# TianyiFranklinWang/MIRROR

Hardware: AMD Instinct MI355X
Metric: SSL samples/sec (slide+RNA pairs) (higher is better)
Workload: dtype bf16; 1 GPU; BASELINE c2: B=16/GPU x [4096 patch tokens x 1024-d] + [2048 genes], D=512, RNA depth 6 / 8 heads, train mode, local-batch InfoNCE; precision_policy=bf16, per_gpu_batch=16, global_batch=16, parallelism=dp1, grad_bucket_dtype=f32, step_launch=hip_graph

## Files before the change

include/mirror_hip.h:

```cpp
#ifndef MIRROR_HIP_H
#define MIRROR_HIP_H
#include <stdint.h>

#ifdef __cplusplus
extern "C" {
#endif

#define MH_OK 0
#define MH_EINVAL (-1)
#define MH_EUNSUP (-2)
#define MH_EHIP (-3)

#define MH_F32 0
#define MH_BF16 1

#define MH_ACT_NONE 0
#define MH_ACT_RELU 1
#define MH_ACT_GELU 2

typedef void* mh_stream;

const char* mh_last_error(void);
int mh_version(void);
int mh_exp_build(void);
// ... 95 lines not shown
                        int dt_x, int dt_dy, int dt_dx, int accumulate_dx, float* workspace, int64_t ws_floats,
                        const void* gadd, int pad, int l, void* relu_out, int relu_first, int relu_rows, float* relu_db,
                        const float* row_mask, const float* lm_scale, mh_stream s);

int mh_quant_fp8(const void* x, int64_t n, void* q, float* scale, unsigned* amax_scratch, int dt, mh_stream s);
int mh_quant_fp8_delayed(const void* x, int64_t n, void* q, float* scale, unsigned* ring, const float* tick, float margin,
                         int dt, mh_stream s);
int mh_gemm_fp8(const void* A, int64_t lda, int64_t a_bs, const void* B, int64_t ldb, void* C, int64_t ldc, int64_t c_bs, int batch,
                const float* scale_a, const float* scale_b, const float* bias, int act, int M, int N, int K, int dt_c, mh_stream s);

int mh_softmax_fwd(const void* x, void* y, int64_t rows, int cols, int64_t ldx, int64_t ldy,
                   int dt_x, int dt_y, mh_stream s);
int mh_softmax_bwd(const void* y, const void* dy, void* dx, int64_t rows, int cols, int64_t ldy, int64_t lddy,
                   int64_t lddx, int dt_y, int dt_dy, int dt_dx, mh_stream s);

int mh_softmax_masked_fwd(const void* x, void* y, const float* rowmask, const float* colmask, int64_t batches, int h, int R,
                          int cols, int dt_x, int dt_y, mh_stream s);
int mh_softmax_masked_bwd(const void* y, const void* dy, void* dx, const float* rowmask, const float* colmask, int64_t batches,
                          int h, int R, int cols, int dt_y, int dt_d, mh_stream s);
int mh_row_scale(const void* x, const float* scale, void* y, int64_t rows, int D, int dt, mh_stream s);
int mh_keymask_plan(const unsigned char* mask, float* mrow, float* mlm, float* lscale, int64_t B, int64_t n_src, int lead, int wrap,
                    int pad, int l, mh_stream s);

int mh_landmark_fwd(const void* qkv, void* lm, int B, int n_p, int D, int l, int dt, mh_stream s);
int mh_landmark_bwd(const void* dlm, void* dqkv, int B, int n_p, int D, int l, int dt, mh_stream s);
int mh_resconv_fwd(const void* v, int64_t ldv, int64_t v_bs, const float* w, void* out, int64_t ldo, int64_t o_bs,
                   int B, int n_p, int heads, int dh, int taps, int transpose, int accumulate,
                   int dt_v, int dt_o, mh_stream s);
int mh_resconv_wgrad(const void* v, int64_t ldv, int64_t v_bs, const void* dout, int64_t ldo, int64_t o_bs,
                     float* dw, int B, int n_p, int heads, int dh, int taps, int dt_v, int dt_o, mh_stream s);
int64_t mh_resconv_bwd_workspace_bytes(int B, int n_p, int heads, int dh, int taps);
int mh_resconv_bwd(const void* dout, int64_t ldo, int64_t o_bs, const void* v, int64_t ldv, int64_t v_bs, const float* w, void* dv,
                   int64_t lddv, int64_t dv_bs, float* dw, float* workspace, int64_t ws_floats, int B, int n_p, int heads, int dh,
                   int taps, int dt_v, int dt_o, mh_stream s);
int mh_pinv_absmax(const float* x, uint64_t* stats64, int BH, int m, mh_stream s);
int mh_pinv_z0(const float* x, const uint64_t* stats64, float* z0, int BH, int m, mh_stream s);
int mh_pinv_z0_bwd(const float* x, const float* z0, const float* dz0, const uint64_t* stats64, float* dx,
                   float* scratch1, int scratch_zeroed, int BH, int m, mh_stream s);
int mh_pinv_s2_bwd(const float* p, const float* dz0, const uint64_t* stats64, float* dx, float* scratch1, int scratch_zeroed, int BH,
                   int m, const float* mlm, int heads, mh_stream s);
int mh_pinv_chain_prep(const float* x, const uint64_t* stats64, float* z0, void* xp, void* z0p, int BH, int m, mh_stream s);
int mh_pinv_chain_pack(const float* dz, void* up, int BH, int m, mh_stream s);
int mh_pinv_chain_fwd(const void* XP, void* saved, void* zfT, int BH, int m, int iters, const float* z0f, const uint64_t* stats64,
                      int z0_rowmajor, mh_stream s);
int mh_nys_sim2(const void* lm, float* a2, void* xp, float* z0f, uint64_t* stats64, int B, int m, int D, int heads, float scale,
                int64_t lm_ld, const float* mlm, mh_stream s);
int mh_nys_dz_dav(const float* dw2, const float* av, const void* zfT, void* up, void* dav, float* delta3, int BH, int m, int dh,
                  mh_stream s);
int mh_pinv_chain_bwd(const void* XP, const void* saved, const void* dzf, void* work, float* dX, float* dz0, int BH, int m,
                      int iters, mh_stream s);
int64_t mh_pinv_chain_workspace_bytes(int BH, int m, int iters, int which);
int mh_nys_attn1_fwd(const void* qkv, const void* lm, const void* w2, void* out, float* lse1, const float* mrow, const float* mlm,
                     int B, int h, int n_p, int m, int dh, float scale, int accumulate, int64_t lm_ld, void* o1, mh_stream s);
int mh_nys_attn1_fwd_q8(const void* qkv, const void* lm, const void* w2, void* out, float* lse1, int B, int h, int n_p, int m, int dh,
                        float scale, int accumulate, void* q8, unsigned* ring, const float* tick, float margin, float* q8_scale, void* o1,
                        mh_stream s);
int64_t mh_nys_attn3_ws_floats(int B, int h, int n_p);
int64_t mh_nys_attn3_workspace_bytes(int B, int h, int n_p);
int mh_nys_attn3_fwd(const void* qkv, const void* lm, float* av, float* lse3, float* workspace, int64_t ws_floats,
                     const float* mrow, const float* mlm, int B, int h, int n_p, int m, int dh, float scale, int64_t lm_ld,
                     const float* rc_w, void* rc_out, mh_stream s);
int mh_nys_attn1_bwd(const void* qkv, const void* lm, const void* w2, const void* dout, const float* lse1, const void* o1, float* delta1,
                     void* dqkv, float* dw2, float* dlm, const float* mrow, const float* mlm, int B, int h, int n_p, int m, int dh,
                     float scale, int64_t lm_ld, mh_stream s);
int mh_nys_attn3_bwd(const void* qkv, const void* lm, const float* av, const void* dav, const float* lse3, float* delta3,
                     void* dqkv, float* dlm, const float* mrow, const float* mlm, int B, int h, int n_p, int m, int dh,
                     float scale, int64_t lm_ld, mh_stream s);
int mh_nys_cls_attn(const void* qkv, const void* lm, const void* z, const float* lse3, float* row, const float* mrow, const float* mlm,
                    int B, int h, int n_p, int m, int dh, int cls_row, float scale, int64_t lm_ld, int z_colmajor, int dt,
                    mh_stream s);
int mh_lm_merge(const float* a, const float* b, void* out, int64_t rows, int cols, int64_t out_ld, int zero_cols, mh_stream s);
int mh_eye_minus(const float* P, float* T, float d, int BH, int m, mh_stream s);

int mh_seq_finish(void* seq, const float* cls, int B, int N, int add, int D, int dt, mh_stream s);
int mh_seq_finish_bwd(void* dseq, float* dcls, int B, int N, int add, int D, int dt, mh_stream s);
int mh_ppeg_merge(const float* w7, const float* w5, const float* w3, const float* b7, const float* b5,
                  const float* b3, float* merged, float* bsum, int D, mh_stream s);
int mh_ppeg_fwd(const void* x, void* y, const float* merged, const float* bsum, int B, int S, int D,
                int flip, int dt_x, int dt_y, mh_stream s);
int mh_ppeg_wgrad(const void* x, const void* dout, float* dmerged, float* dbsum, int B, int S, int D,
                  int dt_x, int dt_o, mh_stream s);
int mh_ppeg_bwd(const float* x, const float* dy, const float* merged, float* dx, float* dmerged, float* dbsum, int B, int S,
                int D, void* drop_out, float* drop_db, float p, uint64_t seed, uint64_t offset, const uint64_t* dev_base,
                mh_stream s);
int mh_ppeg_grad_scatter(const float* dmerged, const float* dbsum, float* dw7, float* dw5, float* dw3, float* db7,
                         float* db5, float* db3, int D, mh_stream s);

int mh_rank_mask(const float* noise, float* mask, int B, int N, int len_keep, mh_stream s);
int mh_mask_apply_fwd(const void* x, void* y, const float* mask, const float* token, const float* pos, int B, int T, int D,
                      int first, int token_scalar, int dt_x, int dt_y, mh_stream s);
int mh_mask_apply_bwd_dbias_ok(const void* dy, const void* dx, const float* dpos, int D, int dt_dy, int dt_dx);
int mh_mask_apply_bwd(const void* dy, void* dx, const float* mask, float* dtoken, float* dpos, int B, int T, int D,
                      int first, int token_scalar, int dt_dy, int dt_dx, float* dbias, mh_stream s);

typedef struct {
    int32_t B, D, Hh, H;
    float eps, p_drop;
    uint64_t seed, offset;
    const uint64_t* dev_base;
    const void *w_qkv, *w_proj, *w_fc1, *w_fc2;
    const void *wt_qkv, *wt_proj, *wt_fc1, *wt_fc2;
    const float *b_qkv, *b_proj, *b_fc1, *b_fc2;
    const float *g1, *be1, *g2, *be2;
    const float* x;
    float* y;
    float* stats;
// ... 217 lines not shown
```

mirror_amd/_lib.py:

```python
from __future__ import annotations

import ctypes as C
import os

_HERE = os.path.dirname(os.path.abspath(__file__))
LIB_PATH = os.environ.get("MIRROR_HIP_LIB") or os.path.join(_HERE, "lib", "libmirror_hip.so")

MH_F32, MH_BF16 = 0, 1
ACT_NONE, ACT_RELU, ACT_GELU = 0, 1, 2


class GemmEpi(C.Structure):
    _fields_ = [
        ("kind", C.c_int32), ("resid", C.c_void_p),
        ("p", C.c_float), ("seed", C.c_uint64), ("offset", C.c_uint64), ("dev_base", C.c_void_p),
        ("mask", C.c_void_p), ("token", C.c_void_p), ("pos", C.c_void_p),
        ("rows_per_batch", C.c_int32), ("first", C.c_int32),
        ("tgt", C.c_void_p), ("tgt_bs", C.c_int64), ("sq", C.c_void_p),
    ]


class SkinnyWgradItem(C.Structure):
    _fields_ = [("dy", C.c_void_p), ("lddy", C.c_int64), ("x", C.c_void_p), ("ldx", C.c_int64), ("dw", C.c_void_p), ("lddw", C.c_int64),
                ("db", C.c_void_p), ("M", C.c_int32), ("N", C.c_int32), ("K", C.c_int32), ("dt_dy", C.c_int32), ("dt_x", C.c_int32)]
# ... 53 lines not shown
        ("g_total", C.c_void_p), ("g_terms", C.c_void_p),
        ("d_wsi_emb", C.c_void_p), ("d_rna_emb", C.c_void_p), ("d_logit_scale", C.c_void_p), ("d_align_ext", C.c_void_p),
        ("d_rna_pred", C.c_void_p), ("d_rna_tgt", C.c_void_p), ("d_w_mu", C.c_void_p), ("d_w_logstd", C.c_void_p), ("d_r_mu", C.c_void_p),
        ("d_r_logstd", C.c_void_p), ("d_w_score", C.c_void_p), ("d_r_score", C.c_void_p),
    ]


class RnaBlockDesc(C.Structure):
    _fields_ = (
        [("B", C.c_int32), ("D", C.c_int32), ("Hh", C.c_int32), ("H", C.c_int32), ("eps", C.c_float), ("p_drop", C.c_float),
         ("seed", C.c_uint64), ("offset", C.c_uint64), ("dev_base", C.c_void_p)]
        + [(n, C.c_void_p) for n in (
            "w_qkv", "w_proj", "w_fc1", "w_fc2", "wt_qkv", "wt_proj", "wt_fc1", "wt_fc2",
            "b_qkv", "b_proj", "b_fc1", "b_fc2", "g1", "be1", "g2", "be2",
            "x", "y", "stats", "qkv", "attn", "o", "x1", "u", "f", "dy", "dx",
            "dw_qkv", "dw_proj", "dw_fc1", "dw_fc2", "db_qkv", "db_proj", "db_fc1", "db_fc2", "dg1", "dbe1", "dg2", "dbe2",
            "scratch")])


_SIGS = {
    "mh_gemm": [C.POINTER(GemmDesc)],
    "mh_skinny_fwd": [P, L, P, L, P, P, L, P, L, I, I, I, I, I, I],
    "mh_skinny_wgrad": [P, L, P, L, P, L, P, I, I, I, I, I, I],
    "mh_skinny_wgrad_many": [C.POINTER(SkinnyWgradItem), I],
    "mh_transpose_bf16": [P, P, I, I],
    "mh_transpose_bf16_many": [P, P, P, I, I, I, I],
    "mh_layernorm_fwd": [P, P, P, P, P, P, I, I, I, L, L, F, I, I],
    "mh_layernorm_fwd_dual": [P, P, P, P, P, P, P, I, I, I, L, L, F],
    "mh_layernorm_fwd_q8": [P, P, P, P, P, P, I, I, I, L, L, F, P, P, P, F, P],
    "mh_layernorm_bwd": [P, P, P, P, P, P, P, P, I, I, I, L, L, I, I, I, I, P, L],
    "mh_layernorm_bwd_fan": [P, P, P, P, P, P, P, P, I, I, I, L, L, I, I, P, L, P, F, P],
    "mh_layernorm_bwd_drop": [P, P, P, P, P, P, P, P, I, I, I, L, L, I, I, P, L, P, F, P, P, F, U64, U64, P, P, I],
    "mh_layernorm_bwd_lm": [P, P, P, P, P, P, P, P, I, I, I, L, L, I, I, I, I, P, L, P, I, I, P, I, I, P, P, P],
    "mh_layernorm_fwd_lm": [P, P, P, P, P, P, P, P, I, I, I, L, I, I, F, P, P],
    "mh_softmax_fwd": [P, P, L, I, L, L, I, I],
    "mh_softmax_bwd": [P, P, P, L, I, L, L, L, I, I, I],
    "mh_landmark_fwd": [P, P, I, I, I, I, I],
    "mh_landmark_bwd": [P, P, I, I, I, I, I],
    "mh_resconv_fwd": [P, L, L, P, P, L, L, I, I, I, I, I, I, I, I, I],
    "mh_resconv_wgrad": [P, L, L, P, L, L, P, I, I, I, I, I, I, I],
    "mh_resconv_bwd": [P, L, L, P, L, L, P, P, L, L, P, P, L, I, I, I, I, I, I, I],
    "mh_pinv_absmax": [P, P, I, I],
    "mh_pinv_z0": [P, P, P, I, I],
    "mh_pinv_z0_bwd": [P, P, P, P, P, P, I, I, I],
    "mh_pinv_s2_bwd": [P, P, P, P, P, I, I, I, P, I],
    "mh_eye_minus": [P, P, F, I, I],
    "mh_pinv_chain_prep": [P, P, P, P, P, I, I],
    "mh_pinv_chain_pack": [P, P, I, I],
    "mh_pinv_chain_fwd": [P, P, P, I, I, I, P, P, I],
    "mh_nys_sim2": [P, P, P, P, P, I, I, I, I, F, L, P],
    "mh_nys_dz_dav": [P, P, P, P, P, P, I, I, I],
    "mh_pinv_chain_bwd": [P, P, P, P, P, P, I, I, I],
    "mh_nys_attn1_fwd": [P, P, P, P, P, P, P, I, I, I, I, I, F, I, L, P],
    "mh_nys_attn1_fwd_q8": [P, P, P, P, P, I, I, I, I, I, F, I, P, P, P, F, P, P],
    "mh_nys_attn3_fwd": [P, P, P, P, P, L, P, P, I, I, I, I, I, F, L, P, P],
    "mh_nys_attn1_bwd": [P, P, P, P, P, P, P, P, P, P, P, P, I, I, I, I, I, F, L],
    "mh_nys_attn3_bwd": [P, P, P, P, P, P, P, P, P, P, I, I, I, I, I, F, L],
    "mh_nys_cls_attn": [P, P, P, P, P, P, P, I, I, I, I, I, I, F, L, I, I],
    "mh_seq_finish": [P, P, I, I, I, I, I],
    "mh_seq_finish_bwd": [P, P, I, I, I, I, I],
    "mh_ppeg_merge": [P, P, P, P, P, P, P, P, I],
    "mh_ppeg_fwd": [P, P, P, P, I, I, I, I, I, I],
    "mh_ppeg_wgrad": [P, P, P, P, I, I, I, I, I],
    "mh_ppeg_bwd": [P, P, P, P, P, P, I, I, I, P, P, F, U64, U64, P],
    "mh_ppeg_grad_scatter": [P, P, P, P, P, P, P, P, I],
    "mh_rank_mask": [P, P, I, I, I],
    "mh_mask_apply_fwd": [P, P, P, P, P, I, I, I, I, I, I, I],
    "mh_mask_apply_bwd": [P, P, P, P, P, I, I, I, I, I, I, I, P],
    "mh_headattn_fwd": [P, P, P, I, I, I, I],
    "mh_headattn_bwd": [P, P, P, P, I, I, I, I],
    "mh_add": [P, P, P, L, I, I, I],
    "mh_lm_merge": [P, P, P, L, I, L, I],
    "mh_cast": [P, P, L, I, I],
    "mh_gelu_fwd": [P, P, L, I, I],
    "mh_gelu_bwd": [P, P, P, L, I, I, I],
    "mh_relu_bwd": [P, P, P, L, I, L, L, L, I, I, I],
    "mh_dropout": [P, P, L, F, U64, U64, P, I, I],
    "mh_noise_draws": [P, L, L, U64, U64, P],
    "mh_dropout_add": [P, P, P, L, F, U64, U64, P, I],
    "mh_dropout_lite": [P, P, P, L, F, U64, U64, P, I, I],
    "mh_timestamp": [P],
    "mh_dropout_lite_colsum": [P, P, L, I, F, U64, U64, P, P],
    "mh_colsum": [P, P, L, I, L, I],
    "mh_l2norm_fwd": [P, P, P, I, I, L, F, I, I],
    "mh_l2norm_bwd": [P, P, P, P, I, I, L, F, I, I, I, I],
    "mh_exp_fwd": [P, P, L],
    "mh_exp_bwd": [P, P, P, L, I],
    "mh_reparam_fwd": [P, P, P, P, L],
    "mh_reparam_bwd": [P, P, P, P, P, P, P, L],
    "mh_ce_rows_fwd": [P, L, P, F, I, I, I, F, P, P, P],
    "mh_ce_rows_bwd": [P, L, P, F, P, P, I, F, P, P, I, I, I],
    "mh_mse_masked_fwd": [P, P, P, P, L, I, L, L, I, I],
    "mh_mse_masked_fwd_ordered": [P, P, P, P, L, I, L, L, I, I, P],
    "mh_mse_masked_bwd": [P, P, P, P, P, F, P, P, L, I, L, L, I, I, I, P, I],
    "mh_fanout_bwd": [P, P, F, P, P, I, I, I, I],
    "mh_gather_rows": [P, P, P, L, L, L, I],
    "mh_sample_rows": [P, P, P, P, I, I, L, U64, U64, P, F],
    "mh_sample_weighted": [P, L, P, L, U64, U64, P],
    "mh_quant_fp8": [P, L, P, P, P, I],
    "mh_quant_fp8_delayed": [P, L, P, P, P, P, F, I],
    "mh_gemm_fp8": [P, L, L, P, L, P, L, L, I, P, P, P, I, I, I, I, I],
    "mh_weighted_sum": [P, P, P, P, P, P, F, F, F, F, F, F, I, P],
    "mh_weighted_sum_bwd": [P, F, F, F, F, F, F, I, P],
    "mh_softmax_masked_fwd": [P, P, P, P, L, I, I, I, I, I],
    "mh_softmax_masked_bwd": [P, P, P, P, P, L, I, I, I, I, I],
    "mh_row_scale": [P, P, P, L, I, I],
# ... 145 lines not shown
```

mirror_amd/csrc/nystrom_fused.hip:

```cpp
#include <cstdlib>
#include <cstring>
#include "gemm_kernel.h"

namespace {

constexpr int NM = 256;
constexpr int ND = 64;
constexpr int NP = 72;
constexpr int NT = 256;
constexpr int TR = 128;

typedef __attribute__((address_space(3))) s16x4 lds_s16x4;
typedef short s16x8 __attribute__((ext_vector_type(8)));

__device__ __forceinline__ bf16x8 frag_kc(const bf16_t* img, int row0, int k0, int lane) {
    return *reinterpret_cast<const bf16x8*>(img + (row0 + (lane & 31)) * NP + k0 + 8 * (lane >> 5));
}
template <int PITCH = NP>
__device__ __forceinline__ bf16x8 frag_tr(const bf16_t* img, int col0, int kb, int lane) {
    const int g16 = lane >> 4, i = lane & 15, q = i >> 2, p = i & 3;
    const bf16_t* a0 = img + (kb + 4 * (g16 >> 1) + q) * PITCH + col0 + 16 * (g16 & 1) + 4 * p;
    s16x4 lo = __builtin_amdgcn_ds_read_tr16_b64_v4i16((lds_s16x4*)a0);
    s16x4 hi = __builtin_amdgcn_ds_read_tr16_b64_v4i16((lds_s16x4*)(a0 + 8 * PITCH));
    s16x8 v = __builtin_shufflevector(lo, hi, 0, 1, 2, 3, 4, 5, 6, 7);
// ... 78 lines not shown
__device__ __forceinline__ void tile_store(const u32x4 (&regs)[ROWS * 8 / NT], bf16_t* img, int tid) {
#pragma unroll
    for (int i = 0; i < ROWS * 8 / NT; i++) {
        const int cid = tid + i * NT, r = cid >> 3, c = cid & 7;
        *reinterpret_cast<u32x4*>(img + r * NP + c * 8) = regs[i];
    }
}
__device__ __forceinline__ void store_row8(bf16_t* p, const f32x16& a, int hl) {
    unsigned w[4][2];
#pragma unroll
    for (int g = 0; g < 4; g++) {
        w[g][0] = pack_bf2(a[4 * g + 0], a[4 * g + 1]);
        w[g][1] = pack_bf2(a[4 * g + 2], a[4 * g + 3]);
    }
#pragma unroll
    for (int pr = 0; pr < 2; pr++) {
        const u32x2 s0 = __builtin_amdgcn_permlane32_swap(w[2 * pr][0], w[2 * pr + 1][0], false, false);
        const u32x2 s1 = __builtin_amdgcn_permlane32_swap(w[2 * pr][1], w[2 * pr + 1][1], false, false);
        const u32x4 v = {s0[0], s1[0], s0[1], s1[1]};
        *reinterpret_cast<u32x4*>(p + 8 * (2 * pr + hl)) = v;
    }
}

constexpr float NEG_FILL = -1.0e6f;
__device__ __forceinline__ void mask_fill16(f32x16& l2, const f32x16& vr, float vl) {
#pragma unroll
    for (int e = 0; e < 16; e++) l2[e] = (vr[e] * vl != 0.f) ? l2[e] : NEG_FILL;
}
__device__ __forceinline__ void mask_zero16(f32x16& d, const f32x16& vr, float vl) {
#pragma unroll
    for (int e = 0; e < 16; e++) d[e] = (vr[e] * vl != 0.f) ? d[e] : 0.f;
}

struct Q8Out {
    unsigned char* q;
    unsigned* ring;
    const float* tick;
    float margin;
    float* scale;
};

struct Geo {
    int h, n_p, D;
    float scale, scale2;
    const float* mrow;
    const float* mlm;
    int accumulate;
    long lm_ld;
    const float* rc_w;
    bf16_t* rc_out;
};
constexpr int RC_TAPS = 33, RC_HALO = 16;

template <bool MASKED, bool Q8 = false>
__global__ __launch_bounds__(NT) void nys_a1_fwd_kernel(const bf16_t* __restrict__ qkv, const bf16_t* __restrict__ lm,
                                                        const bf16_t* __restrict__ w2, bf16_t* __restrict__ out,
                                                        float* __restrict__ lse1, Geo g, Q8Out q8 = Q8Out{}, bf16_t* __restrict__ o1 = nullptr) {
    __shared__ __attribute__((aligned(16))) bf16_t s_kl_[NM * NP];
    __shared__ __attribute__((aligned(16))) bf16_t s_w2_[NM * NP];
    __shared__ __attribute__((aligned(16))) float s_mlm_[NM];
    const int tid = threadIdx.x, lane = tid & 63, wave = tid >> 6, c = lane & 31, hl = lane >> 5;
    const int bh = blockIdx.y, b = bh / g.h, hd = bh % g.h, D = g.D;
    const long LD = g.lm_ld;
    float q8mul = 1.f, q8max = 0.f;
    int q8cur = 0;
    if constexpr (Q8) {
        const int t = (int)q8.tick[0];
        q8cur = t % 3;
        const float amax = __uint_as_float(q8.ring[(t + 2) % 3]) * q8.margin;
        q8mul = amax > 0.f ? 448.f / amax : 1.f;
        if (blockIdx.x == 0 && blockIdx.y == 0 && tid == 0) {
            q8.scale[0] = amax > 0.f ? amax / 448.f : 1.f;
            q8.ring[(t + 1) % 3] = 0u;
        }
    }
    stage_rows<NM>(s_kl_, lm + (long)b * NM * LD + D + hd * ND, LD, tid);
    stage_rows<NM>(s_w2_, w2 + (long)bh * NM * ND, ND, tid);
    constexpr bool masked = MASKED;
    s_mlm_[tid] = masked ? g.mlm[(long)b * NM + tid] : 1.f;
    const int nblk = g.n_p / 32, stride = 4 * gridDim.x;
    int rb = 4 * blockIdx.x + wave;
    const bf16_t* qb = qkv + (long)b * g.n_p * 3 * D + hd * ND;
    bf16x8 qn[4];
    if (rb < nblk) {
#pragma unroll
        for (int ks = 0; ks < 4; ks++) qn[ks] = frag_g(qb + (long)(32 * rb + c) * 3 * D, 16 * ks, lane);
    }
    __syncthreads();
#pragma unroll 1
    for (; rb < nblk; rb += stride) {
        const long row = 32L * rb + c;
        int opq = 0;
        asm volatile("" : "+v"(opq));
        const bf16_t* s_kl = s_kl_ + opq;
        const bf16_t* s_w2 = s_w2_ + opq;
        const float* s_mlm = s_mlm_ + opq;
        const float mr = masked ? g.mrow[(long)b * g.n_p + row] : 1.f;
        bf16x8 qf[4];
#pragma unroll
        for (int ks = 0; ks < 4; ks++) qf[ks] = qn[ks];
        if (rb + stride < nblk) {
#pragma unroll
            for (int ks = 0; ks < 4; ks++) qn[ks] = frag_g(qb + (long)(32 * (rb + stride) + c) * 3 * D, 16 * ks, lane);
        }
        bf16_t* orow = out + ((long)b * g.n_p + row) * D + hd * ND;
        u32x2 old[2][4];
        if (g.accumulate) {
#pragma unroll
            for (int nb = 0; nb < 2; nb++)
#pragma unroll
                for (int gq = 0; gq < 4; gq++) old[nb][gq] = *reinterpret_cast<const u32x2*>(orow + 32 * nb + 8 * gq + 4 * hl);
        }
        float mrun = NEG_BIG, lrun = 0.f;
        f32x16 o[2] = {zero16(), zero16()};
        f32x16 snext = zero16();
#pragma unroll
        for (int ks = 0; ks < 4; ks++) snext = MFMA(frag_kc(s_kl, 0, 16 * ks, lane), qf[ks], snext);
#pragma unroll
        for (int blk = 0; blk < 8; blk++) {
            f32x16 sb = snext;
            if (blk + 1 < 8) {
                snext = zero16();
#pragma unroll
                for (int ks = 0; ks < 4; ks++) snext = MFMA(frag_kc(s_kl, 32 * (blk + 1), 16 * ks, lane), qf[ks], snext);
            }
            float sc2 = g.scale2;
            if (masked) {
                sb = sb * g.scale2;
                mask_fill16(sb, rowvals16(s_mlm + 32 * blk, hl), mr);
                sc2 = 1.f;
            }
            float mx = vmax16(sb);
            mx = fmaxf(mx, __shfl_xor(mx, 32, 64));
            const float mnew = fmaxf(mrun, mx * sc2);
            if (__builtin_amdgcn_ballot_w64(mnew != mrun)) {
                const float alpha = __builtin_amdgcn_exp2f(mrun - mnew);
                lrun *= alpha;
                o[0] *= alpha;
                o[1] *= alpha;
                mrun = mnew;
            }
// ... 495 lines not shown
            *reinterpret_cast<u32x2*>(prow + 24) = u32x2{pw1[2], pw1[3]};
            *reinterpret_cast<u32x2*>(drow) = u32x2{dw0[0], dw0[1]};
            *reinterpret_cast<u32x2*>(drow + 8) = u32x2{dw0[2], dw0[3]};
            *reinterpret_cast<u32x2*>(drow + 16) = u32x2{dw1[0], dw1[1]};
            *reinterpret_cast<u32x2*>(drow + 24) = u32x2{dw1[2], dw1[3]};
        }
        __syncthreads();
        if (more) {
            *reinterpret_cast<u32x4*>(s_k + kr * NP + kc * 8) = rk;
            if (tid < HT) s_mr[tid] = masked ? g.mrow[(long)b * g.n_p + (long)(ht + 1) * HT + tid] : 1.f;
        }
        f32x16 a2 = zero16();
#pragma unroll
        for (int t = 0; t < NM / 16; t++) a2 = MFMA(frag_tr(a_img, 32 * dhalf, 16 * t, lane), frag_tr(b_img, 32 * kb2, 16 * t, lane), a2);
        store_row8(dqkv + ((long)b * g.n_p + (long)ht * HT + 32 * kb2 + c) * 3 * D + (isk ? D : 2 * D) + hd * ND + 32 * dhalf, a2, hl);
        __syncthreads();
    }
    float* dqb = dlm + (long)b * NM * 2 * D + hd * ND;
#pragma unroll
    for (int nb = 0; nb < 2; nb++) atomic_tile(dqb + (long)(32 * wave) * 2 * D + 32 * nb, 2 * D, accq[nb], hl, c);
}

int pick_walkers(int BH, int n_p) {
    int w = 1;
    while (BH * w < 512 && 4 * w * 2 <= n_p / 32) w *= 2;
    return w;
}

#define NYS_LAUNCH(kern, grid, block, shm, stream, ...)                                              \
    do {                                                                                             \
        if (g.mrow) hipLaunchKernelGGL((kern<true>), grid, block, shm, stream, __VA_ARGS__);        \
        else hipLaunchKernelGGL((kern<false>), grid, block, shm, stream, __VA_ARGS__);              \
    } while (0)

int check_geo(const char* fn, int B, int h, int n_p, int m, int dh) {
    MH_REQUIRE(m == NM && dh == ND, "%s: built for m = %d landmarks and dh = %d (got m=%d dh=%d); other shapes use mh_gemm + mh_softmax",
               fn, NM, ND, m, dh);
    MH_REQUIRE(B >= 0 && h >= 1 && n_p >= NM && n_p % NM == 0, "%s: n_p=%d must be a positive multiple of %d", fn, n_p, NM);
    return MH_OK;
}

}

extern "C" int mh_nys_attn1_fwd(const void* qkv, const void* lm, const void* w2, void* out, float* lse1, const float* mrow,
                                const float* mlm, int B, int h, int n_p, int m, int dh, float scale, int accumulate, int64_t lm_ld, void* o1,
                                mh_stream s) {
    if (int e = check_geo("mh_nys_attn1_fwd", B, h, n_p, m, dh)) return e;
    MH_REQUIRE(lm_ld == 0 || (lm_ld >= 2L * h * ND && lm_ld % 8 == 0), "mh_nys_attn1_fwd: lm_ld must be 0 or a multiple of 8 >= 2 D");
    if (B == 0) return MH_OK;
    MH_REQUIRE((mrow == nullptr) == (mlm == nullptr), "mh_nys_attn1_fwd: mrow and mlm go together");
    const Geo g{h, n_p, h * ND, scale, scale * LOG2E, mrow, mlm, accumulate, lm_ld > 0 ? lm_ld : 2L * h * ND, nullptr, nullptr};
    MH_REQUIRE((((uintptr_t)o1) & 15) == 0, "mh_nys_attn1_fwd: o1 must be 16-byte aligned");
    NYS_LAUNCH(nys_a1_fwd_kernel, dim3(pick_walkers(B * h, n_p), B * h), dim3(NT), 0, (hipStream_t)s, (const bf16_t*)qkv, (const bf16_t*)lm,
                       (const bf16_t*)w2, (bf16_t*)out, lse1, g, Q8Out{}, (bf16_t*)o1);
    MH_LAUNCH_CHECK("mh_nys_attn1_fwd");
    return MH_OK;
}

extern "C" int mh_nys_attn1_fwd_q8(const void* qkv, const void* lm, const void* w2, void* out, float* lse1, int B, int h, int n_p, int m,
                                   int dh, float scale, int accumulate, void* q8, unsigned* ring, const float* tick, float margin,
                                   float* q8_scale, void* o1, mh_stream s) {
    if (int e = check_geo("mh_nys_attn1_fwd_q8", B, h, n_p, m, dh)) return e;
    if (B == 0) return MH_OK;
    MH_REQUIRE(q8 && ring && tick && q8_scale && margin >= 1.f && ((uintptr_t)q8 & 3) == 0, "mh_nys_attn1_fwd_q8: q8, ring, tick, scale and margin >= 1");
    const Geo g{h, n_p, h * ND, scale, scale * LOG2E, nullptr, nullptr, accumulate, 2L * h * ND, nullptr, nullptr};
    const Q8Out o{(unsigned char*)q8, ring, tick, margin, q8_scale};
    hipLaunchKernelGGL((nys_a1_fwd_kernel<false, true>), dim3(pick_walkers(B * h, n_p), B * h), dim3(NT), 0, (hipStream_t)s, (const bf16_t*)qkv,
                       (const bf16_t*)lm, (const bf16_t*)w2, (bf16_t*)out, lse1, g, o, (bf16_t*)o1);
    MH_LAUNCH_CHECK("mh_nys_attn1_fwd_q8");
    return MH_OK;
}

int pick_splits(int BH, int ntiles);

extern "C" int64_t mh_nys_attn3_ws_floats(int B, int h, int n_p) {
    if (B <= 0 || h <= 0 || n_p < TR) return 0;
    const int splits = pick_splits(B * h, n_p / TR);
    return splits > 1 ? (int64_t)B * h * splits * A3_PART : 0;
}

extern "C" int64_t mh_nys_attn3_workspace_bytes(int B, int h, int n_p) { return 4 * mh_nys_attn3_ws_floats(B, h, n_p); }

extern "C" int mh_nys_attn3_fwd(const void* qkv, const void* lm, float* av, float* lse3, float* workspace, int64_t ws_floats,
                                const float* mrow, const float* mlm, int B, int h, int n_p, int m, int dh, float scale, int64_t lm_ld,
                                const float* rc_w, void* rc_out, mh_stream s) {
    if (int e = check_geo("mh_nys_attn3_fwd", B, h, n_p, m, dh)) return e;
    MH_REQUIRE(lm_ld == 0 || (lm_ld >= 2L * h * ND && lm_ld % 8 == 0), "mh_nys_attn3_fwd: lm_ld must be 0 or a multiple of 8 >= 2 D");
    MH_REQUIRE((rc_w == nullptr) == (rc_out == nullptr) && (((uintptr_t)rc_out) & 15) == 0, "mh_nys_attn3_fwd: rc_w and rc_out (16-byte aligned) go together");
    if (B == 0) return MH_OK;
    const Geo g{h, n_p, h * ND, scale, scale * LOG2E, mrow, mlm, 0, lm_ld > 0 ? lm_ld : 2L * h * ND, rc_w, (bf16_t*)rc_out};
    const int ntiles = n_p / TR;
    int splits = pick_splits(B * h, ntiles);
    if (!workspace || ws_floats < (int64_t)B * h * splits * A3_PART) splits = 1;
    const int tpw = (ntiles + splits - 1) / splits;
    splits = (ntiles + tpw - 1) / tpw;
    if (rc_w) {
        if (g.mrow) hipLaunchKernelGGL((nys_a3_fwd_kernel<true, true>), dim3(splits, B * h), dim3(NT), 0, (hipStream_t)s, (const bf16_t*)qkv,
                                       (const bf16_t*)lm, av, lse3, workspace, g, tpw);
        else hipLaunchKernelGGL((nys_a3_fwd_kernel<false, true>), dim3(splits, B * h), dim3(NT), 0, (hipStream_t)s, (const bf16_t*)qkv,
                                (const bf16_t*)lm, av, lse3, workspace, g, tpw);
    } else {
        NYS_LAUNCH(nys_a3_fwd_kernel, dim3(splits, B * h), dim3(NT), 0, (hipStream_t)s, (const bf16_t*)qkv, (const bf16_t*)lm, av,
                           lse3, workspace, g, tpw);
    }
    MH_LAUNCH_CHECK("mh_nys_attn3_fwd");
    if (splits > 1) {
        hipLaunchKernelGGL(nys_a3_combine_kernel, dim3(ND / 16, B * h), dim3(NM), 0, (hipStream_t)s, (const float*)workspace, av, lse3,
                           splits);
        MH_LAUNCH_CHECK("mh_nys_attn3_fwd(combine)");
    }
    return MH_OK;
}

int pick_splits(int BH, int ntiles) {
    int splits = 1;
    while (BH * splits < 256 && splits * 2 <= ntiles) splits *= 2;
    return splits;
}

extern "C" int mh_nys_attn1_bwd(const void* qkv, const void* lm, const void* w2, const void* dout, const float* lse1, const void* o1,
                                float* delta1, void* dqkv, float* dw2, float* dlm, const float* mrow, const float* mlm, int B, int h,
// ... 32 lines not shown
```

mirror_amd/functional.py:

```python
from __future__ import annotations

from dataclasses import dataclass
from typing import List, Optional, Tuple

import os

import torch
from torch.autograd import Function

from . import kernels as K
from ._lib import ACT_NONE, ACT_RELU, MH_BF16, MH_F32

f32, bf16 = torch.float32, torch.bfloat16


@dataclass(frozen=True)
class Precision:
    name: str
    mma: int
    act: torch.dtype
    pinv_mma: int
    fp8_fwd: bool = False


# ... 1670 lines not shown
                z0, xt = K.pinv_chain_prep(a2, st, K.pinv_chain_z0_slot(chain_saved))
            zfT = torch.empty((Bn, h, m_l, m_l), device=qkv.device, dtype=bf16)
            zf = zfT.transpose(-1, -2)
            side = _side_stream(qkv.device)
            side.wait_stream(torch.cuda.current_stream())
            with torch.cuda.stream(side):
                if one:
                    K.nys_sim2(lm, h, scale, st, out=(a2, xt), mlm=mlm_s2)
                    K.pinv_chain_fwd(xt, chain_saved, zfT, iters, z0f=a2, stats=st, z0_rowmajor=True)
                else:
                    K.pinv_chain_fwd(xt, chain_saved, zfT, iters)
            saved = [(xt, chain_saved, z0 if z0 is not None else st)]
            ctx.z0_stored = z0 is not None
            K.shared_chip = True
        tile = (not chain) and pm == MH_BF16 and K.gemm_tile_ok(m_l, m_l, m_l)
        if tile and _TILE_SIDE:
            side = _side_stream(qkv.device)
            side.wait_stream(torch.cuda.current_stream())
            with torch.cuda.stream(side):
                zf, saved, st, ctx.a2b = pinv_forward_tile(a2, iters, want_a2b=True)
        if link is not None:
            link.core = True
            link.run("v_cols")
        fused = K.nys_fused_ok(qkv, h, m_l) and lm.dtype == bf16
        lse1 = lse3 = a1 = a3 = None
        out = torch.empty((Bn, n_p, D), device=qkv.device, dtype=A)
        rc_in_a3 = fused and _RC_FUSED and A == bf16 and res_w.numel() == h * 33
        if fused:
            av, lse3 = K.nys_attn3_fwd(qkv, lm, h, scale, kmask,
                                       rc=(res_w.detach().reshape(-1).contiguous(), out) if rc_in_a3 else None)
        else:
            sm1 = (kmask is None and A == bf16 and mma == MH_BF16 and q.dtype == bf16
                   and K.gemm_softmax_ok(n_p, lm.shape[1], dh, q.dtype, kl.dtype))
            if sm1:
                a1 = K.gemm(q, kl.transpose(-1, -2), alpha=scale, mma=mma, out_dtype=bf16, softmax=True)
            else:
                a1 = K.gemm(q, kl.transpose(-1, -2), alpha=scale, mma=mma, out_dtype=f32)
            a3 = K.gemm(ql, k.transpose(-1, -2), alpha=scale, mma=mma, out_dtype=f32)
            if kmask is None:
                if not sm1:
                    a1 = K.softmax_fwd(a1, a1 if A == f32 else None, out_dtype=A)
                a3 = K.softmax_fwd(a3, a3 if A == f32 else None, out_dtype=A)
            else:
                a1 = K.softmax_masked_fwd(a1, mrow, mlm, a1 if A == f32 else None, out_dtype=A)
                a3 = K.softmax_masked_fwd(a3, mlm, mrow, a3 if A == f32 else None, out_dtype=A)
        if tile and not _TILE_SIDE:
            zf, saved, st, ctx.a2b = pinv_forward_tile(a2, iters, want_a2b=True)
        elif not chain and not tile:
            zf, saved, st = pinv_forward(a2, iters, pm, sd)
        if not fused:
            av = K.gemm(a3, v, mma=mma, out_dtype=f32)
        pio = pm if (pm == MH_BF16 or A == f32) else mma
        w2 = None
        if side is not None and fused:
            w2 = torch.empty((Bn, h, m_l, dh), device=qkv.device, dtype=A)
            av_ready = torch.cuda.current_stream().record_event()
            with torch.cuda.stream(side):
                side.wait_event(av_ready)
                K.gemm(zf, av, out=w2, mma=pio)
        if fused and not rc_in_a3:
            K.resconv(qkv[..., 2 * D:], res_w.detach().contiguous(), out, h, transpose=False, accumulate=False)
        if side is not None:
            torch.cuda.current_stream().wait_stream(side)
            if chain:
                K.shared_chip = False
        if w2 is None:
            w2 = K.gemm(zf, av, mma=pio, out_dtype=A)
        o1 = None
        if fused:
            o1 = torch.empty_like(out)
            st8 = _fp8_state
            site = st8["sites"].get(q8_key) if (q8_key is not None and st8["tick"] is not None and kmask is None) else None
            if site is not None and st8["host_step"] - site[1] >= 2:
                q8 = torch.empty(out.shape, device=out.device, dtype=torch.uint8)
                lse1, sc8 = K.nys_attn1_fwd_q8(qkv, lm, w2, out, h, scale, True, q8, site[0], st8["tick"], o1=o1)
                q8_out.append((q8, sc8))
            else:
                lse1 = K.nys_attn1_fwd(qkv, lm, w2, out, h, scale, accumulate=True, kmask=kmask, o1=o1)
        else:
            K.gemm(a1, w2, out=_heads(out, 0, 1, h), mma=mma)
            K.resconv(qkv[..., 2 * D:], res_w.detach().contiguous(), out, h, transpose=False, accumulate=True)
        stats = (lse1, lse3) if fused else (a1, a3)
        if link is not None and link.capture is not None:
            link.capture.update(qkv=qkv, lm=lm, z=zfT if chain else (zf if zf.dtype == f32 else K.cast(zf, f32)), z_colmajor=bool(chain),
                                lse3=lse3 if fused else None, kmask=kmask, heads=h, scale=scale)
        ctx.has_o1 = o1 is not None
        ctx.save_for_backward(qkv, res_w, lm, stats[0], a2, stats[1], av, w2, st, zfT if chain else zf,
                              *([o1] if o1 is not None else []), *[t for it in saved for t in it])
        ctx.cfg = (heads, l, prec)
        ctx.chain = (chain, iters, fused)
        ctx.tile = tile
        ctx.kmask, ctx.link = kmask, link
        return out

    @staticmethod
    def backward(ctx, dout):
        qkv, res_w, lm, a1, a2, a3, av, w2, st, zf, *flat = ctx.saved_tensors
        o1 = None
        if ctx.has_o1:
            o1, flat = flat[0], flat[1:]
        chain, iters, fused = ctx.chain
        kmask = ctx.kmask
        if kmask is not None:
            mrow, mlm, lscale = kmask
        sm_bwd = (lambda y, dy, rm, cm: K.softmax_bwd(y, dy)) if kmask is None else K.softmax_masked_bwd
        zfT = zf if chain else None
        if chain:
            zf = zf.transpose(-1, -2)
        saved = None if chain else [tuple(flat[i:i + 4]) for i in range(0, len(flat), 4)]
        heads, l, prec = ctx.cfg
        A, mma, pm = prec.act, prec.mma, prec.pinv_mma
        Bn, n_p, D3 = qkv.shape
        D, h = D3 // 3, heads
        dh = D // h
        m = n_p // l
        scale = dh ** -0.5
        tr = lambda t: t.transpose(-1, -2)
        dout = dout.contiguous()
        if dout.dtype != A:
            dout = K.cast(dout, A)
        q, k, v = (_heads(qkv, i, 3, h) for i in range(3))
        ql, kl = _heads(lm, 0, 2, h), _heads(lm, 1, 2, h)
        dO = _heads(dout, 0, 1, h)
        de = dlm_out = None
        if ctx.lm_ext and A == bf16:
            de, dqkv, dlm_out = ext_rows_alloc(Bn, n_p, m, D3, 2 * D, qkv.device)
        else:
            dqkv = torch.empty_like(qkv)
        dq, dk, dv = (_heads(dqkv, i, 3, h) for i in range(3))
# ... 803 lines not shown
```

mirror_amd/kernels.py:

```python
from __future__ import annotations

import ctypes as C
import functools
import os
from typing import Optional


import torch

from . import _lib
from ._lib import ACT_GELU, ACT_NONE, ACT_RELU, MH_BF16, MH_F32, GemmDesc, MirrorHipError

_DT = {torch.float32: MH_F32, torch.bfloat16: MH_BF16}


def dt(t: torch.Tensor) -> int:
    try:
        return _DT[t.dtype]
    except KeyError:
        raise MirrorHipError(f"unsupported dtype {t.dtype} (f32 / bf16 only)") from None


_raw_stream = getattr(torch._C, "_cuda_getCurrentRawStream", None)

# ... 908 lines not shown

def _nys_check(name: str, B: int, h: int, n_p: int, **tensors) -> None:
    D = h * NYS_FUSED_DH
    want = {"qkv": ((B, n_p, 3 * D), torch.bfloat16), "dqkv": ((B, n_p, 3 * D), torch.bfloat16),
            "lm": ((B, NYS_FUSED_M, 2 * D), torch.bfloat16), "dlm": ((B, NYS_FUSED_M, 2 * D), torch.float32),
            "w2": ((B, h, NYS_FUSED_M, NYS_FUSED_DH), torch.bfloat16), "dw2": ((B, h, NYS_FUSED_M, NYS_FUSED_DH), torch.float32),
            "av": ((B, h, NYS_FUSED_M, NYS_FUSED_DH), torch.float32), "dav": ((B, h, NYS_FUSED_M, NYS_FUSED_DH), torch.bfloat16),
            "out": ((B, n_p, D), torch.bfloat16), "dout": ((B, n_p, D), torch.bfloat16), "o1": ((B, n_p, D), torch.bfloat16),
            "lse1": ((B, h, n_p), torch.float32), "delta1": ((B, h, n_p), torch.float32),
            "lse3": ((B, h, NYS_FUSED_M), torch.float32)}
    for k, t in tensors.items():
        shape, dtype = want[k]
        if k == "lm" and tuple(t.shape) == shape and t.dtype == dtype and _lm_ld(t) > 0:
            continue
        if tuple(t.shape) != shape or t.dtype != dtype or not t.is_contiguous():
            raise MirrorHipError(f"{name}: {k} must be contiguous {dtype} {shape}, got {t.dtype} {tuple(t.shape)} "
                                 f"contiguous={t.is_contiguous()}")


def _lm_ld(lm: torch.Tensor) -> int:
    if lm.dim() != 3 or lm.stride(2) != 1 or lm.stride(0) != lm.shape[1] * lm.stride(1) or lm.stride(1) < lm.shape[2] or lm.stride(1) % 8:
        return 0
    return int(lm.stride(1))


def _nys_launch(name: str, flops: float, fn) -> None:
    if gemm_profiler is None:
        fn()
    else:
        gemm_profiler.launch_named(name, flops, fn)


def _nys_masks(kmask, B: int, n_p: int):
    if kmask is None:
        return None, None
    mrow, mlm = kmask[0], kmask[1]
    _chk(mrow, mlm)
    assert mrow.shape == (B, n_p) and mlm.shape == (B, NYS_FUSED_M) and mrow.dtype == mlm.dtype == torch.float32
    assert mrow.is_contiguous() and mlm.is_contiguous()
    return _p(mrow), _p(mlm)


def nys_attn1_fwd(qkv, lm, w2, out, heads: int, scale: float, accumulate: bool = False, kmask=None, o1=None) -> torch.Tensor:
    _chk(qkv, lm, w2, out, o1)
    B, n_p, _ = qkv.shape
    lse1 = torch.empty((B, heads, n_p), device=qkv.device, dtype=torch.float32)
    _nys_check("nys_attn1_fwd", B, heads, n_p, qkv=qkv, lm=lm, w2=w2, out=out, **({} if o1 is None else {"o1": o1}))
    _nys_launch("nys_a1_fwd_kernel", 2 * 2.0 * n_p * NYS_FUSED_M * NYS_FUSED_DH * B * heads,
                lambda: _lib.call("mh_nys_attn1_fwd", _p(qkv), _p(lm), _p(w2), _p(out), _p(lse1), *_nys_masks(kmask, B, n_p), B, heads,
                                  n_p, NYS_FUSED_M, NYS_FUSED_DH, scale, int(accumulate), _lm_ld(lm), _p(o1), stream=_stream()))
    return lse1


def nys_attn1_fwd_q8(qkv, lm, w2, out, heads: int, scale: float, accumulate: bool, q8, ring, tick, margin: float = 1.25, o1=None):
    _chk(qkv, lm, w2, out, q8, ring, tick)
    B, n_p, _ = qkv.shape
    if not (q8.dtype == torch.uint8 and q8.shape == out.shape and q8.is_contiguous() and ring.dtype == torch.int32 and ring.numel() == 3
            and tick.dtype == torch.float32):
        raise MirrorHipError("nys_attn1_fwd_q8: q8 uint8 shaped like out, int32[3] ring, f32 tick")
    lse1 = torch.empty((B, heads, n_p), device=qkv.device, dtype=torch.float32)
    sc = torch.empty((1,), device=qkv.device, dtype=torch.float32)
    _chk(o1)
    _nys_check("nys_attn1_fwd", B, heads, n_p, qkv=qkv, lm=lm.contiguous(), w2=w2, out=out, **({} if o1 is None else {"o1": o1}))
    lm = lm.contiguous()
    _nys_launch("nys_a1_fwd_kernel", 2 * 2.0 * n_p * NYS_FUSED_M * NYS_FUSED_DH * B * heads,
                lambda: _lib.call("mh_nys_attn1_fwd_q8", _p(qkv), _p(lm), _p(w2), _p(out), _p(lse1), B, heads, n_p, NYS_FUSED_M,
                                  NYS_FUSED_DH, scale, int(accumulate), _p(q8), _p(ring), _p(tick), float(margin), _p(sc), _p(o1),
                                  stream=_stream()))
    return lse1, sc


def nys_attn3_fwd(qkv, lm, heads: int, scale: float, kmask=None, rc=None):
    _chk(qkv, lm)
    B, n_p, _ = qkv.shape
    rc_w = rc_out = None
    if rc is not None:
        rc_w, rc_out = rc
        _chk(rc_w, rc_out)
        if (rc_w.dtype != torch.float32 or rc_w.numel() != heads * 33 or not rc_w.is_contiguous() or rc_out.dtype != torch.bfloat16
                or tuple(rc_out.shape) != (B, n_p, heads * NYS_FUSED_DH) or not rc_out.is_contiguous()):
            raise MirrorHipError("nys_attn3_fwd: rc = (f32 [h * 33] filters, contiguous bf16 [B, n_p, D] output)")
    av = torch.empty((B, heads, NYS_FUSED_M, NYS_FUSED_DH), device=qkv.device, dtype=torch.float32)
    lse3 = torch.empty((B, heads, NYS_FUSED_M), device=qkv.device, dtype=torch.float32)
    _nys_check("nys_attn3_fwd", B, heads, n_p, qkv=qkv, lm=lm)
    nws = int(_lib.load().mh_nys_attn3_ws_floats(B, heads, n_p))
    ws = torch.empty((nws,), device=qkv.device, dtype=torch.float32) if nws else None
    _nys_launch("nys_a3_fwd_kernel", 2 * 2.0 * n_p * NYS_FUSED_M * NYS_FUSED_DH * B * heads,
                lambda: _lib.call("mh_nys_attn3_fwd", _p(qkv), _p(lm), _p(av), _p(lse3), _p(ws), nws, *_nys_masks(kmask, B, n_p), B,
                                  heads, n_p, NYS_FUSED_M, NYS_FUSED_DH, scale, _lm_ld(lm), _p(rc_w), _p(rc_out), stream=_stream()))
    return av, lse3


NYS_CLS_GEOMETRIES = ((64, 256), (96, 384))


def nys_cls_attn(qkv, lm, z, heads: int, scale: float, cls_row: int, lse3=None, mrow=None, mlm=None, z_colmajor: bool = False):
    if qkv.dim() != 3 or lm.dim() != 3 or qkv.shape[2] % (3 * heads) or qkv.dtype != lm.dtype:
        raise MirrorHipError(f"nys_cls_attn: qkv [B, n_p, 3D] and lm [B, m, 2D] of one dtype, D a multiple of heads={heads}; got "
                             f"{tuple(qkv.shape)} {qkv.dtype}, {tuple(lm.shape)} {lm.dtype}")
    B, n_p, D3 = qkv.shape
    D, m = D3 // 3, lm.shape[1]
    dh = D // heads
    if (dh, m) not in NYS_CLS_GEOMETRIES:
        raise MirrorHipError(f"nys_cls_attn: built for (dh, m) in {NYS_CLS_GEOMETRIES}, got ({dh}, {m})")
    if tuple(lm.shape) != (B, m, 2 * D) or n_p < m or n_p % m:
        raise MirrorHipError(f"nys_cls_attn: lm must be [{B}, m, {2 * D}] and n_p={n_p} a multiple of m={m}; lm is {tuple(lm.shape)}")
# ... 1178 lines not shown
```

Before: 2201 samples/s.

## Fuse z·av product into Nystrom attn1 forward kernel prologue

Adds a ZAV variant of the Nystrom attn1 forward kernel. Each block computes w2 = zf·av for its head in its prologue with MFMA, streaming the zfT chunks through the k_l shared-memory image with double-buffered register prefetch. The first walker block per head writes w2 back to global memory for the backward pass. This removes the separate w2 GEMM (and any side-stream overlap) and its global round trip, at the cost of every walker block recomputing the 256x256x64 product redundantly. The grid is also remapped so blocks of the same head group cluster together.

```diff
diff --git a/include/mirror_hip.h b/include/mirror_hip.h
--- a/include/mirror_hip.h
+++ b/include/mirror_hip.h
@@ -171,6 +171,9 @@
 int64_t mh_pinv_chain_workspace_bytes(int BH, int m, int iters, int which);
 int mh_nys_attn1_fwd(const void* qkv, const void* lm, const void* w2, void* out, float* lse1, const float* mrow, const float* mlm,
                      int B, int h, int n_p, int m, int dh, float scale, int accumulate, int64_t lm_ld, void* o1, mh_stream s);
+int mh_nys_attn1_fwd_zav(const void* qkv, const void* lm, const void* zfT, const float* av, void* w2, void* out, float* lse1,
+                         const float* mrow, const float* mlm, int B, int h, int n_p, int m, int dh, float scale, int accumulate,
+                         int64_t lm_ld, void* o1, mh_stream s);
 int mh_nys_attn1_fwd_q8(const void* qkv, const void* lm, const void* w2, void* out, float* lse1, int B, int h, int n_p, int m, int dh,
                         float scale, int accumulate, void* q8, unsigned* ring, const float* tick, float margin, float* q8_scale, void* o1,
                         mh_stream s);
diff --git a/mirror_amd/_lib.py b/mirror_amd/_lib.py
--- a/mirror_amd/_lib.py
+++ b/mirror_amd/_lib.py
@@ -129,6 +129,7 @@
     "mh_nys_dz_dav": [P, P, P, P, P, P, I, I, I],
     "mh_pinv_chain_bwd": [P, P, P, P, P, P, I, I, I],
     "mh_nys_attn1_fwd": [P, P, P, P, P, P, P, I, I, I, I, I, F, I, L, P],
+    "mh_nys_attn1_fwd_zav": [P, P, P, P, P, P, P, P, P, I, I, I, I, I, F, I, L, P],
     "mh_nys_attn1_fwd_q8": [P, P, P, P, P, I, I, I, I, I, F, I, P, P, P, F, P, P],
     "mh_nys_attn3_fwd": [P, P, P, P, P, L, P, P, I, I, I, I, I, F, L, P, P],
     "mh_nys_attn1_bwd": [P, P, P, P, P, P, P, P, P, P, P, P, I, I, I, I, I, F, L],
diff --git a/mirror_amd/csrc/nystrom_fused.hip b/mirror_amd/csrc/nystrom_fused.hip
--- a/mirror_amd/csrc/nystrom_fused.hip
+++ b/mirror_amd/csrc/nystrom_fused.hip
@@ -154,15 +154,33 @@
 };
 constexpr int RC_TAPS = 33, RC_HALO = 16;
 
-template <bool MASKED, bool Q8 = false>
+struct ZavIn {
+    const bf16_t* zfT;
+    const float* av;
+    bf16_t* w2;
+};
+constexpr int ZR = 64;
+constexpr int ZP = 288;
+static_assert(ZR * ZP <= NM * NP && NM % ZR == 0 && ZR * NM / 8 % NT == 0, "a chunk of zfT fits the k_l image");
+
+template <bool MASKED, bool Q8 = false, bool ZAV = false>
 __global__ __launch_bounds__(NT) void nys_a1_fwd_kernel(const bf16_t* __restrict__ qkv, const bf16_t* __restrict__ lm,
                                                         const bf16_t* __restrict__ w2, bf16_t* __restrict__ out,
-                                                        float* __restrict__ lse1, Geo g, Q8Out q8 = Q8Out{}, bf16_t* __restrict__ o1 = nullptr) {
+                                                        float* __restrict__ lse1, Geo g, Q8Out q8 = Q8Out{}, bf16_t* __restrict__ o1 = nullptr,
+                                                        ZavIn zv = ZavIn{}) {
     __shared__ __attribute__((aligned(16))) bf16_t s_kl_[NM * NP];
     __shared__ __attribute__((aligned(16))) bf16_t s_w2_[NM * NP];
     __shared__ __attribute__((aligned(16))) float s_mlm_[NM];
     const int tid = threadIdx.x, lane = tid & 63, wave = tid >> 6, c = lane & 31, hl = lane >> 5;
-    const int bh = blockIdx.y, b = bh / g.h, hd = bh % g.h, D = g.D;
+    int bh = blockIdx.y, wk = blockIdx.x;
+    if constexpr (ZAV) {
+        if (gridDim.y % 8 == 0) {
+            const int lin = blockIdx.x + gridDim.x * blockIdx.y, per = 8 * gridDim.x, r = lin % per;
+            bh = 8 * (lin / per) + (r & 7);
+            wk = r >> 3;
+        }
+    }
+    const int b = bh / g.h, hd = bh % g.h, D = g.D;
     const long LD = g.lm_ld;
     float q8mul = 1.f, q8max = 0.f;
     int q8cur = 0;
@@ -176,12 +194,74 @@
             q8.ring[(t + 1) % 3] = 0u;
         }
     }
-    stage_rows<NM>(s_kl_, lm + (long)b * NM * LD + D + hd * ND, LD, tid);
-    stage_rows<NM>(s_w2_, w2 + (long)bh * NM * ND, ND, tid);
+    if constexpr (ZAV) {
+        const float* avb = zv.av + (long)bh * NM * ND;
+        const bf16_t* zb = zv.zfT + (long)bh * NM * NM;
+#pragma unroll
+        for (int i = 0; i < NM * ND / 4 / NT; i++) {
+            const int cid = tid + i * NT, r = cid >> 4, q = cid & 15;
+            const f32x4 x = *reinterpret_cast<const f32x4*>(avb + r * ND + 4 * q);
+            *reinterpret_cast<u32x2*>(s_w2_ + r * NP + 4 * q) = u32x2{pack_bf2(x[0], x[1]), pack_bf2(x[2], x[3])};
+        }
+        constexpr int ZN = ZR * NM / 8 / NT;
+        u32x4 zr[2][ZN], klr[NM * 8 / NT];
+#pragma unroll
+        for (int jc = 0; jc < 2; jc++)
+#pragma unroll
+            for (int i = 0; i < ZN; i++) {
+                const int cid = tid + i * NT, r = cid >> 5, q = cid & 31;
+                zr[jc][i] = *reinterpret_cast<const u32x4*>(zb + (long)(ZR * jc + r) * NM + 8 * q);
+            }
+        f32x16 acc[2][2] = {{zero16(), zero16()}, {zero16(), zero16()}};
+#pragma unroll
+        for (int jc = 0; jc < NM / ZR; jc++) {
+            if (jc > 0) __syncthreads();
+#pragma unroll
+            for (int i = 0; i < ZN; i++) {
+                const int cid = tid + i * NT, r = cid >> 5, q = cid & 31;
+                *reinterpret_cast<u32x4*>(s_kl_ + r * ZP + 8 * q) = zr[jc & 1][i];
+            }
+            if (jc + 2 < NM / ZR) {
+#pragma unroll
+                for (int i = 0; i < ZN; i++) {
+                    const int cid = tid + i * NT, r = cid >> 5, q = cid & 31;
+                    zr[jc & 1][i] = *reinterpret_cast<const u32x4*>(zb + (long)(ZR * (jc + 2) + r) * NM + 8 * q);
+                }
+            } else if (jc + 2 == NM / ZR) {
+                tile_load<NM>(klr, lm + (long)b * NM * LD + D + hd * ND, LD, tid);
+            }
+            __syncthreads();
+#pragma unroll
+            for (int t = 0; t < ZR / 16; t++) {
+                bf16x8 zf[2], af[2];
+#pragma unroll
+                for (int lb = 0; lb < 2; lb++) zf[lb] = frag_tr<ZP>(s_kl_, 64 * wave + 32 * lb, 16 * t, lane);
+#pragma unroll
+                for (int nb = 0; nb < 2; nb++) af[nb] = frag_tr(s_w2_, 32 * nb, ZR * jc + 16 * t, lane);
+#pragma unroll
+                for (int lb = 0; lb < 2; lb++)
+#pragma unroll
+                    for (int nb = 0; nb < 2; nb++) acc[lb][nb] = MFMA(af[nb], zf[lb], acc[lb][nb]);
+            }
+        }
+        __syncthreads();
+#pragma unroll
+        for (int lb = 0; lb < 2; lb++)
+#pragma unroll
+            for (int nb = 0; nb < 2; nb++)
+#pragma unroll
+                for (int gq = 0; gq < 4; gq++)
+                    *reinterpret_cast<u32x2*>(s_w2_ + (64 * wave + 32 * lb + c) * NP + 32 * nb + 8 * gq + 4 * hl) =
+                        u32x2{pack_bf2(acc[lb][nb][4 * gq], acc[lb][nb][4 * gq + 1]), pack_bf2(acc[lb][nb][4 * gq + 2], acc[lb][nb][4 * gq + 3])};
+        tile_store<NM>(klr, s_kl_, tid);
+    } else {
+        stage_rows<NM>(s_kl_, lm + (long)b * NM * LD + D + hd * ND, LD, tid);
+        stage_rows<NM>(s_w2_, w2 + (long)bh * NM * ND, ND, tid);
+    }
     constexpr bool masked = MASKED;
     s_mlm_[tid] = masked ? g.mlm[(long)b * NM + tid] : 1.f;
     const int nblk = g.n_p / 32, stride = 4 * gridDim.x;
-    int rb = 4 * blockIdx.x + wave;
+    int rb = 4 * wk + wave;
     const bf16_t* qb = qkv + (long)b * g.n_p * 3 * D + hd * ND;
     bf16x8 qn[4];
     if (rb < nblk) {
@@ -189,6 +269,16 @@
         for (int ks = 0; ks < 4; ks++) qn[ks] = frag_g(qb + (long)(32 * rb + c) * 3 * D, 16 * ks, lane);
     }
     __syncthreads();
+    if constexpr (ZAV) {
+        if (wk == 0) {
+            bf16_t* wb = zv.w2 + (long)bh * NM * ND;
+#pragma unroll
+            for (int i = 0; i < NM * 8 / NT; i++) {
+                const int cid = tid + i * NT, r = cid >> 3, cc = cid & 7;
+                *reinterpret_cast<u32x4*>(wb + r * ND + cc * 8) = *reinterpret_cast<const u32x4*>(s_w2_ + r * NP + cc * 8);
+            }
+        }
+    }
 #pragma unroll 1
     for (; rb < nblk; rb += stride) {
         const long row = 32L * rb + c;
@@ -790,8 +880,28 @@
     const Geo g{h, n_p, h * ND, scale, scale * LOG2E, mrow, mlm, accumulate, lm_ld > 0 ? lm_ld : 2L * h * ND, nullptr, nullptr};
     MH_REQUIRE((((uintptr_t)o1) & 15) == 0, "mh_nys_attn1_fwd: o1 must be 16-byte aligned");
     NYS_LAUNCH(nys_a1_fwd_kernel, dim3(pick_walkers(B * h, n_p), B * h), dim3(NT), 0, (hipStream_t)s, (const bf16_t*)qkv, (const bf16_t*)lm,
-                       (const bf16_t*)w2, (bf16_t*)out, lse1, g, Q8Out{}, (bf16_t*)o1);
+                       (const bf16_t*)w2, (bf16_t*)out, lse1, g, Q8Out{}, (bf16_t*)o1, ZavIn{});
     MH_LAUNCH_CHECK("mh_nys_attn1_fwd");
+    return MH_OK;
+}
+
+extern "C" int mh_nys_attn1_fwd_zav(const void* qkv, const void* lm, const void* zfT, const float* av, void* w2, void* out, float* lse1,
+                                    const float* mrow, const float* mlm, int B, int h, int n_p, int m, int dh, float scale, int accumulate,
+                                    int64_t lm_ld, void* o1, mh_stream s) {
+    if (int e = check_geo("mh_nys_attn1_fwd_zav", B, h, n_p, m, dh)) return e;
+    MH_REQUIRE(lm_ld == 0 || (lm_ld >= 2L * h * ND && lm_ld % 8 == 0), "mh_nys_attn1_fwd_zav: lm_ld must be 0 or a multiple of 8 >= 2 D");
+    if (B == 0) return MH_OK;
+    MH_REQUIRE((mrow == nullptr) == (mlm == nullptr), "mh_nys_attn1_fwd_zav: mrow and mlm go together");
+    MH_REQUIRE(zfT && av && w2 && ((((uintptr_t)zfT) | ((uintptr_t)av) | ((uintptr_t)w2) | ((uintptr_t)o1)) & 15) == 0,
+               "mh_nys_attn1_fwd_zav: zfT, av and w2 are needed; they and o1 must be 16-byte aligned");
+    const Geo g{h, n_p, h * ND, scale, scale * LOG2E, mrow, mlm, accumulate, lm_ld > 0 ? lm_ld : 2L * h * ND, nullptr, nullptr};
+    const ZavIn zv{(const bf16_t*)zfT, av, (bf16_t*)w2};
+    const dim3 grid(pick_walkers(B * h, n_p), B * h);
+    if (g.mrow) hipLaunchKernelGGL((nys_a1_fwd_kernel<true, false, true>), grid, dim3(NT), 0, (hipStream_t)s, (const bf16_t*)qkv, (const bf16_t*)lm,
+                                   (const bf16_t*)nullptr, (bf16_t*)out, lse1, g, Q8Out{}, (bf16_t*)o1, zv);
+    else hipLaunchKernelGGL((nys_a1_fwd_kernel<false, false, true>), grid, dim3(NT), 0, (hipStream_t)s, (const bf16_t*)qkv, (const bf16_t*)lm,
+                            (const bf16_t*)nullptr, (bf16_t*)out, lse1, g, Q8Out{}, (bf16_t*)o1, zv);
+    MH_LAUNCH_CHECK("mh_nys_attn1_fwd_zav");
     return MH_OK;
 }
 
@@ -804,7 +914,7 @@
     const Geo g{h, n_p, h * ND, scale, scale * LOG2E, nullptr, nullptr, accumulate, 2L * h * ND, nullptr, nullptr};
     const Q8Out o{(unsigned char*)q8, ring, tick, margin, q8_scale};
     hipLaunchKernelGGL((nys_a1_fwd_kernel<false, true>), dim3(pick_walkers(B * h, n_p), B * h), dim3(NT), 0, (hipStream_t)s, (const bf16_t*)qkv,
-                       (const bf16_t*)lm, (const bf16_t*)w2, (bf16_t*)out, lse1, g, o, (bf16_t*)o1);
+                       (const bf16_t*)lm, (const bf16_t*)w2, (bf16_t*)out, lse1, g, o, (bf16_t*)o1, ZavIn{});
     MH_LAUNCH_CHECK("mh_nys_attn1_fwd_q8");
     return MH_OK;
 }
diff --git a/mirror_amd/functional.py b/mirror_amd/functional.py
--- a/mirror_amd/functional.py
+++ b/mirror_amd/functional.py
@@ -1746,7 +1746,13 @@
             av = K.gemm(a3, v, mma=mma, out_dtype=f32)
         pio = pm if (pm == MH_BF16 or A == f32) else mma
         w2 = None
-        if side is not None and fused:
+        st8 = _fp8_state
+        site = st8["sites"].get(q8_key) if (fused and q8_key is not None and st8["tick"] is not None and kmask is None) else None
+        a1_q8 = site is not None and st8["host_step"] - site[1] >= 2
+        a1_zav = chain and fused and pio == MH_BF16 and not a1_q8
+        if a1_zav:
+            w2 = torch.empty((Bn, h, m_l, dh), device=qkv.device, dtype=A)
+        elif side is not None and fused:
             w2 = torch.empty((Bn, h, m_l, dh), device=qkv.device, dtype=A)
             av_ready = torch.cuda.current_stream().record_event()
             with torch.cuda.stream(side):
@@ -1763,12 +1769,12 @@
         o1 = None
         if fused:
             o1 = torch.empty_like(out)
-            st8 = _fp8_state
-            site = st8["sites"].get(q8_key) if (q8_key is not None and st8["tick"] is not None and kmask is None) else None
-            if site is not None and st8["host_step"] - site[1] >= 2:
+            if a1_q8:
                 q8 = torch.empty(out.shape, device=out.device, dtype=torch.uint8)
                 lse1, sc8 = K.nys_attn1_fwd_q8(qkv, lm, w2, out, h, scale, True, q8, site[0], st8["tick"], o1=o1)
                 q8_out.append((q8, sc8))
+            elif a1_zav:
+                lse1 = K.nys_attn1_fwd_zav(qkv, lm, zfT, av, w2, out, h, scale, accumulate=True, kmask=kmask, o1=o1)
             else:
                 lse1 = K.nys_attn1_fwd(qkv, lm, w2, out, h, scale, accumulate=True, kmask=kmask, o1=o1)
         else:
diff --git a/mirror_amd/kernels.py b/mirror_amd/kernels.py
--- a/mirror_amd/kernels.py
+++ b/mirror_amd/kernels.py
@@ -984,6 +984,21 @@
     return lse1
 
 
+def nys_attn1_fwd_zav(qkv, lm, zfT, av, w2, out, heads: int, scale: float, accumulate: bool = False, kmask=None, o1=None) -> torch.Tensor:
+    _chk(qkv, lm, zfT, av, w2, out, o1)
+    B, n_p, _ = qkv.shape
+    if tuple(zfT.shape) != (B, heads, NYS_FUSED_M, NYS_FUSED_M) or zfT.dtype != torch.bfloat16 or not zfT.is_contiguous():
+        raise MirrorHipError(f"nys_attn1_fwd_zav: zfT must be contiguous bf16 [{B}, {heads}, {NYS_FUSED_M}, {NYS_FUSED_M}] (the chain's "
+                             f"column-major output), got {zfT.dtype} {tuple(zfT.shape)} contiguous={zfT.is_contiguous()}")
+    lse1 = torch.empty((B, heads, n_p), device=qkv.device, dtype=torch.float32)
+    _nys_check("nys_attn1_fwd_zav", B, heads, n_p, qkv=qkv, lm=lm, av=av, w2=w2, out=out, **({} if o1 is None else {"o1": o1}))
+    _nys_launch("nys_a1_fwd_kernel", 2 * 2.0 * n_p * NYS_FUSED_M * NYS_FUSED_DH * B * heads,
+                lambda: _lib.call("mh_nys_attn1_fwd_zav", _p(qkv), _p(lm), _p(zfT), _p(av), _p(w2), _p(out), _p(lse1),
+                                  *_nys_masks(kmask, B, n_p), B, heads, n_p, NYS_FUSED_M, NYS_FUSED_DH, scale, int(accumulate), _lm_ld(lm),
+                                  _p(o1), stream=_stream()))
+    return lse1
+
+
 def nys_attn1_fwd_q8(qkv, lm, w2, out, heads: int, scale: float, accumulate: bool, q8, ring, tick, margin: float = 1.25, o1=None):
     _chk(qkv, lm, w2, out, q8, ring, tick)
     B, n_p, _ = qkv.shape
```

Measured after the change: 2213 samples/s, median of 3. About the same (+0.6%).
